# Scalsol/mega.pytorch

Hardware: AMD Instinct MI355X
Metric: frames/sec MEGA R-101 inference, 1000x600 VID clip (higher is better)
Workload: dtype bf16

## Files before the change

mega/pytorch_amd/csrc/bneck64.hip:

```cpp
#include <cstdlib>

#include "common.h"

namespace {

constexpr int BK_TY = 8, BK_TX = 16;
constexpr int BK_PY = BK_TY + 2, BK_PX = BK_TX + 2;
constexpr int BK_NP = BK_PY * BK_PX;
constexpr int BK_M1 = 192;
constexpr int BK_NT = 512;
constexpr int BK_W2ROW = 1168;
constexpr int BK_WROW = 144;
constexpr int BK_SBROW = 528;
constexpr int BK_OFF_W2 = 0;
constexpr int BK_OFF_T1 = 64 * BK_W2ROW;
constexpr int BK_OFF_XB = BK_OFF_T1 + BK_NP * 128;
constexpr int BK_OFF_W1 = BK_OFF_XB + BK_M1 * 128;
constexpr int BK_XB_BYTES = 256 * BK_WROW;
constexpr int BK_OFF_T2 = BK_OFF_XB + BK_XB_BYTES;
constexpr int BK_LDS = BK_OFF_T2 + 128 * 128;
constexpr int BK_OFF_ST = BK_OFF_T1;
static_assert(BK_OFF_ST + 128 * BK_SBROW <= BK_LDS, "staging must fit");
static_assert(BK_M1 * 128 + 64 * BK_WROW <= BK_XB_BYTES, "x chunk + w1 chunk must fit the XB region");

struct Bneck64Params {
  const bf16_t* x;
  const bf16_t* w1;
  const bf16_t* w2;
  const bf16_t* w3;
  const float *s1, *b1, *s2, *b2, *s3, *b3;
  bf16_t* out;
  int N, H, W, tiles_y, tiles_x, ntiles;
};

template <typename HT>
__device__ __forceinline__ f32x16_t bk_mma(f32x16_t acc, const uint4& a, const uint4& b) {
  return Half16<HT>::mfma32(__builtin_bit_cast(u32x4_t, a), __builtin_bit_cast(u32x4_t, b), acc);
}

template <typename HT>
__device__ __forceinline__ unsigned bk_relu_pack(float a, float b) {
  const s16x2_t z = {0, 0};
  return __builtin_bit_cast(unsigned, __builtin_elementwise_max(__builtin_bit_cast(s16x2_t, Half16<HT>::pack2(a, b)), z));
}
template <typename HT>
__device__ __forceinline__ bf16_t bk_relu1(float a) {
  const bf16_t h = Half16<HT>::cvt(a);
  return (short)h < 0 ? (bf16_t)0 : h;
}

template <typename HT>
__global__ __launch_bounds__(BK_NT, 2) void bneck64_kernel(Bneck64Params p) {
  extern __shared__ __attribute__((aligned(16))) unsigned char smem[];
  unsigned char* const w2l = smem + BK_OFF_W2;
  unsigned char* const t1l = smem + BK_OFF_T1;
  unsigned char* const xbl = smem + BK_OFF_XB;
  unsigned char* const w1l = smem + BK_OFF_W1;
  unsigned char* const t2l = smem + BK_OFF_T2;
  unsigned char* const sbl = smem + BK_OFF_ST;
  const int tid = threadIdx.x, lane = tid & 63, wave = tid >> 6;
  const int l31 = lane & 31, h = lane >> 5;

  {
    const uint4* wg = reinterpret_cast<const uint4*>(p.w2);
    for (int e = tid; e < 64 * 72; e += BK_NT) {
      const int n = e / 72, c = e - n * 72;
      *reinterpret_cast<uint4*>(w2l + n * BK_W2ROW + c * 16) = wg[e];
    }
  }

  const unsigned xbytes = (unsigned)((size_t)p.N * p.H * p.W * 512);
  const __amdgpu_buffer_rsrc_t rs_x = __builtin_amdgcn_make_buffer_rsrc(const_cast<bf16_t*>(p.x), 0, (int)xbytes, 0x00020000);
  const __amdgpu_buffer_rsrc_t rs_o = __builtin_amdgcn_make_buffer_rsrc(p.out, 0, (int)xbytes, 0x00020000);
  constexpr unsigned OOB = 0x80000000u;

  auto tile_origin = [&](int t, int& n, int& y0, int& x0) {
    const int per_img = p.tiles_y * p.tiles_x;
    n = t / per_img;
    const int r = t - n * per_img;
    const int ty = r / p.tiles_x;
    y0 = ty * BK_TY;
    x0 = (r - ty * p.tiles_x) * BK_TX;
  };

  u32x4_t px[12], pw1[4];
  auto prefetch = [&](int t) {
    int n, y0, x0;
    const bool live = t < p.ntiles;
    tile_origin(live ? t : 0, n, y0, x0);
    unsigned off[3];
#pragma unroll
    for (int i = 0; i < 3; ++i) {
      const int v = tid + BK_NT * i;
      const int row = v >> 3, j = v & 7;
      const int py = row / BK_PX, pxx = row - py * BK_PX;
      const int yy = y0 - 1 + py, xx = x0 - 1 + pxx;
      const bool ok = live && row < BK_NP && (unsigned)yy < (unsigned)p.H && (unsigned)xx < (unsigned)p.W;
      off[i] = ok ? (unsigned)(((n * p.H + yy) * p.W + xx) * 512 + j * 16) : OOB;
    }
#pragma unroll
    for (int kc = 0; kc < 4; ++kc) {
#pragma unroll
      for (int i = 0; i < 3; ++i) {
        px[3 * kc + i] = __builtin_amdgcn_raw_buffer_load_b128(rs_x, off[i], kc * 128, 0);
      }
      pw1[kc] = *reinterpret_cast<const u32x4_t*>(p.w1 + (tid >> 3) * 256 + kc * 64 + (tid & 7) * 8);
    }
  };

  const int r1 = 32 * wave + l31;
  const unsigned a1_base = (unsigned)(r1 * 128), a1_sw = (unsigned)((r1 >> 1) & 7);
  const unsigned b1_base = (unsigned)(l31 * BK_WROW + h * 16);
  const int mb2 = wave >> 1, nb2 = wave & 1;
  const int ay = 2 * mb2 + (l31 >> 4), ax = l31 & 15;
  const unsigned a2_base = (unsigned)((ay * BK_PX + ax) * 128);
  const int b2_off = (32 * nb2 + l31) * BK_W2ROW + h * 16;
  const unsigned a3_base = (unsigned)(l31 * 128), a3_sw = (unsigned)((l31 >> 1) & 7);
  const unsigned b3_base = (unsigned)((32 * wave + l31) * BK_WROW + h * 16);
  const float s1a = p.s1[l31], s1b = p.s1[32 + l31], b1a = p.b1[l31], b1b = p.b1[32 + l31];
  const float s2v = p.s2[32 * nb2 + l31], b2v = p.b2[32 * nb2 + l31];
  const float s3v = p.s3[32 * wave + l31], b3v = p.b3[32 * wave + l31];

  int t = blockIdx.x;
  prefetch(t);
  __syncthreads();
  for (; t < p.ntiles; t += gridDim.x) {
    int n, y0, x0;
    tile_origin(t, n, y0, x0);
    f32x16_t c1a, c1b;
#pragma unroll
    for (int r = 0; r < 16; ++r) { c1a[r] = 0.f; c1b[r] = 0.f; }
#pragma unroll
    for (int kc = 0; kc < 4; ++kc) {
#pragma unroll
      for (int i = 0; i < 3; ++i) {
        const int v = tid + BK_NT * i;
        const int row = v >> 3, j = v & 7;
        *reinterpret_cast<u32x4_t*>(xbl + row * 128 + ((j ^ ((row >> 1) & 7)) * 16)) = px[3 * kc + i];
      }
      *reinterpret_cast<u32x4_t*>(w1l + (tid >> 3) * BK_WROW + (tid & 7) * 16) = pw1[kc];
      __syncthreads();
      if (wave < 6) {
#pragma unroll
        for (int ks = 0; ks < 4; ++ks) {
          const uint4 a = *reinterpret_cast<const uint4*>(xbl + a1_base + (((unsigned)(2 * ks + h) ^ a1_sw) << 4));
          const uint4 b0 = *reinterpret_cast<const uint4*>(w1l + b1_base + ks * 32);
          const uint4 b1 = *reinterpret_cast<const uint4*>(w1l + 32 * BK_WROW + b1_base + ks * 32);
          c1a = bk_mma<HT>(c1a, a, b0);
          c1b = bk_mma<HT>(c1b, a, b1);
        }
      }
      __syncthreads();
    }
    u32x4_t pw3[4];
#pragma unroll
    for (int i = 0; i < 4; ++i) pw3[i] = reinterpret_cast<const u32x4_t*>(p.w3)[tid + BK_NT * i];
    int ho = h, lo = l31;
    asm volatile("" : "+v"(ho), "+v"(lo));
    if (wave < 6) {
#pragma unroll
      for (int r = 0; r < 16; ++r) {
        const int R = 32 * wave + (r & 3) + 8 * (r >> 2) + 4 * ho;
        if (R < BK_NP) {
          const int py = R / BK_PX, pxx = R - py * BK_PX;
          const int yy = y0 - 1 + py, xx = x0 - 1 + pxx;
          const bool in = (unsigned)yy < (unsigned)p.H && (unsigned)xx < (unsigned)p.W;
          const bf16_t ra = bk_relu1<HT>(c1a[r] * s1a + b1a), rb = bk_relu1<HT>(c1b[r] * s1b + b1b);
          const bf16_t va = in ? ra : (bf16_t)0;
          const bf16_t vb = in ? rb : (bf16_t)0;
          unsigned char* base = t1l + R * 128;
          const int sw = (pxx >> 1) & 7;
          *reinterpret_cast<bf16_t*>(base + (((lo >> 3) ^ sw) * 16) + (lo & 7) * 2) = va;
          *reinterpret_cast<bf16_t*>(base + ((((32 + lo) >> 3) ^ sw) * 16) + (lo & 7) * 2) = vb;
        }
      }
    }
#pragma unroll
    for (int i = 0; i < 4; ++i) {
      const int v = tid + BK_NT * i;
      *reinterpret_cast<u32x4_t*>(xbl + (v >> 3) * BK_WROW + (v & 7) * 16) = pw3[i];
    }
    prefetch(t + gridDim.x);
    __syncthreads();
    f32x16_t c2;
#pragma unroll
    for (int r = 0; r < 16; ++r) c2[r] = 0.f;
#pragma unroll
    for (int kh = 0; kh < 3; ++kh)
#pragma unroll
      for (int kw = 0; kw < 3; ++kw)
#pragma unroll
        for (int ks = 0; ks < 4; ++ks) {
          const unsigned sw2 = (unsigned)(((ax + kw) >> 1) & 7);
          const uint4 a = *reinterpret_cast<const uint4*>(t1l + a2_base + (kh * BK_PX + kw) * 128 +
                                                          (((unsigned)(2 * ks + h) ^ sw2) << 4));
          const uint4 b = *reinterpret_cast<const uint4*>(w2l + b2_off + (kh * 3 + kw) * 128 + ks * 32);
          c2 = bk_mma<HT>(c2, a, b);
        }
    {
      const int c = 32 * nb2 + lo;
#pragma unroll
      for (int r = 0; r < 16; ++r) {
        const int P = 32 * mb2 + (r & 3) + 8 * (r >> 2) + 4 * ho;
        *reinterpret_cast<bf16_t*>(t2l + P * 128 + (((c >> 3) ^ ((P >> 1) & 7)) * 16) + (c & 7) * 2) = bk_relu1<HT>(c2[r] * s2v + b2v);
      }
    }
    __syncthreads();
    unsigned pk[4][8];
    {
      uint4 bf[4];
#pragma unroll
      for (int ks = 0; ks < 4; ++ks) bf[ks] = *reinterpret_cast<const uint4*>(xbl + b3_base + ks * 32);
      const int c3ch = 32 * wave + lo;
      const unsigned res_base = (unsigned)(((n * p.H + y0) * p.W + x0 + 4 * ho) * 512 + c3ch * 2);
#pragma unroll
      for (int mb = 0; mb < 4; ++mb) {
        __builtin_amdgcn_sched_barrier(0);
        float rs[16];
#pragma unroll
        for (int r = 0; r < 16; ++r) {
          const int yy = y0 + 2 * mb + (r >> 3), xx = x0 + (r & 3) + 8 * ((r >> 2) & 1) + 4 * ho;
          const unsigned o = (yy < p.H && xx < p.W) ? res_base : OOB;
          const unsigned short q = __builtin_amdgcn_raw_buffer_load_b16(
              rs_x, o, ((2 * mb + (r >> 3)) * p.W + (r & 3) + 8 * ((r >> 2) & 1)) * 512, 0);
          rs[r] = Half16<HT>::one(q);
        }
        f32x16_t c3;
#pragma unroll
        for (int r = 0; r < 16; ++r) c3[r] = 0.f;
#pragma unroll
        for (int ks = 0; ks < 4; ++ks) {
          const uint4 a = *reinterpret_cast<const uint4*>(t2l + mb * 4096 + a3_base + (((unsigned)(2 * ks + h) ^ a3_sw) << 4));
          c3 = bk_mma<HT>(c3, a, bf[ks]);
        }
#pragma unroll
        for (int q = 0; q < 8; ++q) {
          float v0 = c3[2 * q] * s3v + b3v, v1 = c3[2 * q + 1] * s3v + b3v;
          v0 += rs[2 * q];
          v1 += rs[2 * q + 1];
          pk[mb][q] = bk_relu_pack<HT>(v0, v1);
        }
      }
    }
    __syncthreads();
    {
      const int c3ch = 32 * wave + lo;
#pragma unroll
      for (int mb = 0; mb < 4; ++mb)
#pragma unroll
        for (int r = 0; r < 16; ++r) {
          const int P = 32 * mb + (r & 3) + 8 * (r >> 2) + 4 * ho;
          const unsigned v = pk[mb][r >> 1];
          *reinterpret_cast<bf16_t*>(sbl + P * BK_SBROW + c3ch * 2) = (bf16_t)((r & 1) ? (v >> 16) : (v & 0xffffu));
        }
    }
    __syncthreads();
#pragma unroll
    for (int i = 0; i < 8; ++i) {
      const int id = tid + BK_NT * i;
      const int P = id >> 5, cv = id & 31;
      const int yy = y0 + (P >> 4), xx = x0 + (P & 15);
      const uint4 v = *reinterpret_cast<const uint4*>(sbl + P * BK_SBROW + cv * 16);
      const u32x4_t q = {v.x, v.y, v.z, v.w};
      const unsigned o = (yy < p.H && xx < p.W) ? (unsigned)(((n * p.H + yy) * p.W + xx) * 512 + cv * 16) : OOB;
      __builtin_amdgcn_raw_buffer_store_b128(q, rs_o, o, 0, 0);
    }
    __syncthreads();
  }
}

constexpr int BD_OFF_W2 = 0;
constexpr int BD_OFF_T1 = 64 * BK_W2ROW;
constexpr int BD_OFF_XP = BD_OFF_T1 + BK_NP * 128;
constexpr int BD_OFF_WR = BD_OFF_XP + BK_M1 * 128;
constexpr int BD_LDS = BD_OFF_WR + 256 * BK_WROW;
static_assert(BD_OFF_T1 + 128 * BK_SBROW <= BD_LDS, "output staging must fit over t1 / x patch / weight region");

struct Bneck64DsParams {
  const bf16_t* x;
  const bf16_t* w1;
  const bf16_t* w2;
  const bf16_t* w3;
  const bf16_t* wd;
  const float *s1, *b1, *s2, *b2, *s3, *b3, *sd, *bd;
  bf16_t* out;
  int N, H, W, tiles_y, tiles_x, ntiles;
};

template <typename HT>
__global__ __launch_bounds__(BK_NT, 2) void bneck64_ds_kernel(Bneck64DsParams p) {
  extern __shared__ __attribute__((aligned(16))) unsigned char smem[];
  unsigned char* const w2l = smem + BD_OFF_W2;
  unsigned char* const t1l = smem + BD_OFF_T1;
  unsigned char* const t2l = smem + BD_OFF_T1;
  unsigned char* const xpl = smem + BD_OFF_XP;
  unsigned char* const wrl = smem + BD_OFF_WR;
  unsigned char* const sbl = smem + BD_OFF_T1;
  const int tid = threadIdx.x, lane = tid & 63, wave = tid >> 6;
  const int l31 = lane & 31, h = lane >> 5;
  {
    const uint4* wg = reinterpret_cast<const uint4*>(p.w2);
    for (int e = tid; e < 64 * 72; e += BK_NT) {
      const int n = e / 72, c = e - n * 72;
      *reinterpret_cast<uint4*>(w2l + n * BK_W2ROW + c * 16) = wg[e];
    }
  }
  const unsigned xbytes = (unsigned)((size_t)p.N * p.H * p.W * 128), obytes = (unsigned)((size_t)p.N * p.H * p.W * 512);
  const __amdgpu_buffer_rsrc_t rs_x = __builtin_amdgcn_make_buffer_rsrc(const_cast<bf16_t*>(p.x), 0, (int)xbytes, 0x00020000);
  const __amdgpu_buffer_rsrc_t rs_o = __builtin_amdgcn_make_buffer_rsrc(p.out, 0, (int)obytes, 0x00020000);
  constexpr unsigned OOB = 0x80000000u;
  auto tile_origin = [&](int t, int& n, int& y0, int& x0) {
    const int per_img = p.tiles_y * p.tiles_x;
    n = t / per_img;
    const int r = t - n * per_img;
    const int ty = r / p.tiles_x;
    y0 = ty * BK_TY;
    x0 = (r - ty * p.tiles_x) * BK_TX;
  };
  u32x4_t px[3];
  auto prefetch = [&](int t) {
    int n, y0, x0;
    const bool live = t < p.ntiles;
    tile_origin(live ? t : 0, n, y0, x0);
#pragma unroll
    for (int i = 0; i < 3; ++i) {
      const int v = tid + BK_NT * i;
      const int row = v >> 3, j = v & 7;
      const int py = row / BK_PX, pxx = row - py * BK_PX;
      const int yy = y0 - 1 + py, xx = x0 - 1 + pxx;
      const bool ok = live && row < BK_NP && (unsigned)yy < (unsigned)p.H && (unsigned)xx < (unsigned)p.W;
      px[i] = __builtin_amdgcn_raw_buffer_load_b128(rs_x, ok ? (unsigned)(((n * p.H + yy) * p.W + xx) * 128 + j * 16) : OOB, 0, 0);
    }
  };
  const int r1 = 32 * wave + l31;
  const unsigned a1_base = (unsigned)(r1 * 128), a1_sw = (unsigned)((r1 >> 1) & 7);
  const unsigned bw_base = (unsigned)(l31 * BK_WROW + h * 16);
  const int mb2 = wave >> 1, nb2 = wave & 1;
  const int ay = 2 * mb2 + (l31 >> 4), ax = l31 & 15;
  const unsigned a2_base = (unsigned)((ay * BK_PX + ax) * 128);
  const int b2_off = (32 * nb2 + l31) * BK_W2ROW + h * 16;
  const unsigned a3_base = (unsigned)(l31 * 128), a3_sw = (unsigned)((l31 >> 1) & 7);
  const float s1a = p.s1[l31], s1b = p.s1[32 + l31], b1a = p.b1[l31], b1b = p.b1[32 + l31];
  const float s2v = p.s2[32 * nb2 + l31], b2v = p.b2[32 * nb2 + l31];
  const float s3v = p.s3[32 * wave + l31], b3v = p.b3[32 * wave + l31];
  const float sdv = p.sd[32 * wave + l31], bdv = p.bd[32 * wave + l31];

  int t = blockIdx.x;
  prefetch(t);
  __syncthreads();
  for (; t < p.ntiles; t += gridDim.x) {
    int n, y0, x0;
    tile_origin(t, n, y0, x0);
    int ho = h, lo = l31;
    asm volatile("" : "+v"(ho), "+v"(lo));
#pragma unroll
    for (int i = 0; i < 3; ++i) {
      const int v = tid + BK_NT * i;
      const int row = v >> 3, j = v & 7;
      *reinterpret_cast<u32x4_t*>(xpl + row * 128 + ((j ^ ((row >> 1) & 7)) * 16)) = px[i];
    }
    *reinterpret_cast<u32x4_t*>(wrl + (tid >> 3) * BK_WROW + (tid & 7) * 16) =
        *reinterpret_cast<const u32x4_t*>(p.w1 + (tid >> 3) * 64 + (tid & 7) * 8);
    u32x4_t pwd[4];
#pragma unroll
    for (int i = 0; i < 4; ++i) pwd[i] = reinterpret_cast<const u32x4_t*>(p.wd)[tid + BK_NT * i];
    __syncthreads();
    f32x16_t c1a, c1b;
#pragma unroll
    for (int r = 0; r < 16; ++r) { c1a[r] = 0.f; c1b[r] = 0.f; }
    if (wave < 6) {
#pragma unroll
      for (int ks = 0; ks < 4; ++ks) {
        const uint4 a = *reinterpret_cast<const uint4*>(xpl + a1_base + (((unsigned)(2 * ks + h) ^ a1_sw) << 4));
        const uint4 b0 = *reinterpret_cast<const uint4*>(wrl + bw_base + ks * 32);
        const uint4 b1 = *reinterpret_cast<const uint4*>(wrl + 32 * BK_WROW + bw_base + ks * 32);
        c1a = bk_mma<HT>(c1a, a, b0);
        c1b = bk_mma<HT>(c1b, a, b1);
      }
#pragma unroll
      for (int r = 0; r < 16; ++r) {
        const int R = 32 * wave + (r & 3) + 8 * (r >> 2) + 4 * ho;
        if (R < BK_NP) {
          const int py = R / BK_PX, pxx = R - py * BK_PX;
          const int yy = y0 - 1 + py, xx = x0 - 1 + pxx;
          const bool in = (unsigned)yy < (unsigned)p.H && (unsigned)xx < (unsigned)p.W;
          const bf16_t ra = bk_relu1<HT>(c1a[r] * s1a + b1a), rb = bk_relu1<HT>(c1b[r] * s1b + b1b);
          const bf16_t va = in ? ra : (bf16_t)0;
          const bf16_t vb = in ? rb : (bf16_t)0;
          unsigned char* base = t1l + R * 128;
          const int sw = (pxx >> 1) & 7;
          *reinterpret_cast<bf16_t*>(base + (((lo >> 3) ^ sw) * 16) + (lo & 7) * 2) = va;
          *reinterpret_cast<bf16_t*>(base + ((((32 + lo) >> 3) ^ sw) * 16) + (lo & 7) * 2) = vb;
        }
      }
    }
    __syncthreads();
#pragma unroll
    for (int i = 0; i < 4; ++i) {
      const int v = tid + BK_NT * i;
      *reinterpret_cast<u32x4_t*>(wrl + (v >> 3) * BK_WROW + (v & 7) * 16) = pwd[i];
    }
    u32x4_t pw3[4];
#pragma unroll
    for (int i = 0; i < 4; ++i) pw3[i] = reinterpret_cast<const u32x4_t*>(p.w3)[tid + BK_NT * i];
    prefetch(t + gridDim.x);
    f32x16_t c2;
#pragma unroll
    for (int r = 0; r < 16; ++r) c2[r] = 0.f;
#pragma unroll
    for (int kh = 0; kh < 3; ++kh)
#pragma unroll
      for (int kw = 0; kw < 3; ++kw)
#pragma unroll
        for (int ks = 0; ks < 4; ++ks) {
          const unsigned sw2 = (unsigned)(((ax + kw) >> 1) & 7);
          const uint4 a = *reinterpret_cast<const uint4*>(t1l + a2_base + (kh * BK_PX + kw) * 128 +
                                                          (((unsigned)(2 * ks + h) ^ sw2) << 4));
          const uint4 b = *reinterpret_cast<const uint4*>(w2l + b2_off + (kh * 3 + kw) * 128 + ks * 32);
          c2 = bk_mma<HT>(c2, a, b);
        }
    __syncthreads();
    {
      const int c = 32 * nb2 + lo;
#pragma unroll
      for (int r = 0; r < 16; ++r) {
        const int P = 32 * mb2 + (r & 3) + 8 * (r >> 2) + 4 * ho;
        *reinterpret_cast<bf16_t*>(t2l + P * 128 + (((c >> 3) ^ ((P >> 1) & 7)) * 16) + (c & 7) * 2) = bk_relu1<HT>(c2[r] * s2v + b2v);
      }
    }
    unsigned pk[4][8];
    {
      uint4 bf[4];
#pragma unroll
      for (int ks = 0; ks < 4; ++ks) bf[ks] = *reinterpret_cast<const uint4*>(wrl + 32 * wave * BK_WROW + bw_base + ks * 32);
#pragma unroll
      for (int mb = 0; mb < 4; ++mb) {
        const int R = (2 * mb + (l31 >> 4) + 1) * BK_PX + (l31 & 15) + 1;
        const unsigned xa = (unsigned)(R * 128), xs = (unsigned)((R >> 1) & 7);
        f32x16_t cd;
#pragma unroll
        for (int r = 0; r < 16; ++r) cd[r] = 0.f;
#pragma unroll
        for (int ks = 0; ks < 4; ++ks) {
          const uint4 a = *reinterpret_cast<const uint4*>(xpl + xa + (((unsigned)(2 * ks + h) ^ xs) << 4));
          cd = bk_mma<HT>(cd, a, bf[ks]);
        }
#pragma unroll
        for (int q = 0; q < 8; ++q) pk[mb][q] = Half16<HT>::pack2(cd[2 * q] * sdv + bdv, cd[2 * q + 1] * sdv + bdv);
      }
    }
    __syncthreads();
#pragma unroll
    for (int i = 0; i < 4; ++i) {
      const int v = tid + BK_NT * i;
      *reinterpret_cast<u32x4_t*>(wrl + (v >> 3) * BK_WROW + (v & 7) * 16) = pw3[i];
    }
    __syncthreads();
    {
      uint4 bf[4];
#pragma unroll
      for (int ks = 0; ks < 4; ++ks) bf[ks] = *reinterpret_cast<const uint4*>(wrl + 32 * wave * BK_WROW + bw_base + ks * 32);
#pragma unroll
      for (int mb = 0; mb < 4; ++mb) {
        f32x16_t c3;
#pragma unroll
        for (int r = 0; r < 16; ++r) c3[r] = 0.f;
#pragma unroll
        for (int ks = 0; ks < 4; ++ks) {
          const uint4 a = *reinterpret_cast<const uint4*>(t2l + mb * 4096 + a3_base + (((unsigned)(2 * ks + h) ^ a3_sw) << 4));
          c3 = bk_mma<HT>(c3, a, bf[ks]);
        }
#pragma unroll
        for (int q = 0; q < 8; ++q) {
          float v0 = c3[2 * q] * s3v + b3v, v1 = c3[2 * q + 1] * s3v + b3v;
          v0 += Half16<HT>::lo(pk[mb][q]);
          v1 += Half16<HT>::hi(pk[mb][q]);
          pk[mb][q] = bk_relu_pack<HT>(v0, v1);
        }
      }
    }
    __syncthreads();
    {
      const int c3ch = 32 * wave + lo;
#pragma unroll
      for (int mb = 0; mb < 4; ++mb)
#pragma unroll
        for (int r = 0; r < 16; ++r) {
          const int P = 32 * mb + (r & 3) + 8 * (r >> 2) + 4 * ho;
          const unsigned v = pk[mb][r >> 1];
          *reinterpret_cast<bf16_t*>(sbl + P * BK_SBROW + c3ch * 2) = (bf16_t)((r & 1) ? (v >> 16) : (v & 0xffffu));
        }
    }
    __syncthreads();
#pragma unroll
    for (int i = 0; i < 8; ++i) {
      const int id = tid + BK_NT * i;
      const int P = id >> 5, cv = id & 31;
      const int yy = y0 + (P >> 4), xx = x0 + (P & 15);
      const uint4 v = *reinterpret_cast<const uint4*>(sbl + P * BK_SBROW + cv * 16);
      const u32x4_t q = {v.x, v.y, v.z, v.w};
      const unsigned o = (yy < p.H && xx < p.W) ? (unsigned)(((n * p.H + yy) * p.W + xx) * 512 + cv * 16) : OOB;
      __builtin_amdgcn_raw_buffer_store_b128(q, rs_o, o, 0, 0);
    }
    __syncthreads();
  }
}

}

extern "C" int mega_bottleneck64_fwd_dt(const void* x, const void* w1, const float* s1, const float* b1, const void* w2,
                                        const float* s2, const float* b2, const void* w3, const float* s3, const float* b3,
                                        void* out, int N, int H, int W, int dtype, void* stream) {
  mega_clear_error();
  if (dtype != MEGA_BF16 && dtype != MEGA_F16) return MEGA_ERR_ARG;
  if (!x || !w1 || !s1 || !b1 || !w2 || !s2 || !b2 || !w3 || !s3 || !b3 || !out || N <= 0 || H <= 0 || W <= 0) return MEGA_ERR_ARG;
  if ((size_t)N * H * W * 256 * 2 >= 0x7FF00000ull) return MEGA_ERR_ARG;
  Bneck64Params p;
  p.x = (const bf16_t*)x; p.w1 = (const bf16_t*)w1; p.w2 = (const bf16_t*)w2; p.w3 = (const bf16_t*)w3;
  p.s1 = s1; p.b1 = b1; p.s2 = s2; p.b2 = b2; p.s3 = s3; p.b3 = b3;
  p.out = (bf16_t*)out;
  p.N = N; p.H = H; p.W = W;
  p.tiles_y = cdiv(H, BK_TY);
  p.tiles_x = cdiv(W, BK_TX);
  const long tiles = (long)N * p.tiles_y * p.tiles_x;
  if (tiles > 0x7FFFFFFF) return MEGA_ERR_ARG;
  p.ntiles = (int)tiles;
  int cus = 256;
  {
    static int cached[64] = {0};
    int dev = 0, n = 0;
    if (hipGetDevice(&dev) != hipSuccess || dev < 0 || dev >= 64) dev = 0;
    if (!cached[dev]) {
      if (hipDeviceGetAttribute(&n, hipDeviceAttributeMultiprocessorCount, dev) == hipSuccess && n > 0) cached[dev] = n;
      else cached[dev] = 256;
    }
    cus = cached[dev];
  }
  const int grid = (int)(tiles < cus ? tiles : cus);
  if (dtype == MEGA_F16) {
    (void)hipFuncSetAttribute((const void*)bneck64_kernel<f16_t>, hipFuncAttributeMaxDynamicSharedMemorySize, BK_LDS);
    hipLaunchKernelGGL(bneck64_kernel<f16_t>, dim3(grid), dim3(BK_NT), BK_LDS, (hipStream_t)stream, p);
  } else {
    (void)hipFuncSetAttribute((const void*)bneck64_kernel<bf16_t>, hipFuncAttributeMaxDynamicSharedMemorySize, BK_LDS);
    hipLaunchKernelGGL(bneck64_kernel<bf16_t>, dim3(grid), dim3(BK_NT), BK_LDS, (hipStream_t)stream, p);
  }
  return mega_check_launch();
}

extern "C" int mega_bottleneck64_ds_fwd_dt(const void* x, const void* w1, const float* s1, const float* b1, const void* w2,
                                           const float* s2, const float* b2, const void* w3, const float* s3, const float* b3,
                                           const void* wd, const float* sd, const float* bd, void* out, int N, int H, int W,
                                           int dtype, void* stream) {
  mega_clear_error();
  if (dtype != MEGA_BF16 && dtype != MEGA_F16) return MEGA_ERR_ARG;
  if (!x || !w1 || !s1 || !b1 || !w2 || !s2 || !b2 || !w3 || !s3 || !b3 || !wd || !sd || !bd || !out || N <= 0 || H <= 0 || W <= 0)
    return MEGA_ERR_ARG;
  if ((size_t)N * H * W * 256 * 2 >= 0x7FF00000ull) return MEGA_ERR_ARG;
  Bneck64DsParams p;
  p.x = (const bf16_t*)x; p.w1 = (const bf16_t*)w1; p.w2 = (const bf16_t*)w2; p.w3 = (const bf16_t*)w3; p.wd = (const bf16_t*)wd;
  p.s1 = s1; p.b1 = b1; p.s2 = s2; p.b2 = b2; p.s3 = s3; p.b3 = b3; p.sd = sd; p.bd = bd;
  p.out = (bf16_t*)out;
  p.N = N; p.H = H; p.W = W;
  p.tiles_y = cdiv(H, BK_TY);
  p.tiles_x = cdiv(W, BK_TX);
  const long tiles = (long)N * p.tiles_y * p.tiles_x;
  if (tiles > 0x7FFFFFFF) return MEGA_ERR_ARG;
  p.ntiles = (int)tiles;
  int cus = 256;
  {
    static int cached[64] = {0};
    int dev = 0, n = 0;
    if (hipGetDevice(&dev) != hipSuccess || dev < 0 || dev >= 64) dev = 0;
    if (!cached[dev]) {
      if (hipDeviceGetAttribute(&n, hipDeviceAttributeMultiprocessorCount, dev) == hipSuccess && n > 0) cached[dev] = n;
      else cached[dev] = 256;
    }
    cus = cached[dev];
  }
  const int grid = (int)(tiles < cus ? tiles : cus);
  if (dtype == MEGA_F16) {
    (void)hipFuncSetAttribute((const void*)bneck64_ds_kernel<f16_t>, hipFuncAttributeMaxDynamicSharedMemorySize, BD_LDS);
    hipLaunchKernelGGL(bneck64_ds_kernel<f16_t>, dim3(grid), dim3(BK_NT), BD_LDS, (hipStream_t)stream, p);
  } else {
    (void)hipFuncSetAttribute((const void*)bneck64_ds_kernel<bf16_t>, hipFuncAttributeMaxDynamicSharedMemorySize, BD_LDS);
    hipLaunchKernelGGL(bneck64_ds_kernel<bf16_t>, dim3(grid), dim3(BK_NT), BD_LDS, (hipStream_t)stream, p);
  }
  return mega_check_launch();
}
```

Baseline: 902.8.

## Swap MFMA operand order and vectorise epilogues with LDS scale/bias and slab output

Swaps the A/B operands of every MFMA so accumulators come out channel-contiguous per lane. The bf16 epilogues for t1, t2 and the downsample path can then write packed 8-byte words instead of scalar 2-byte stores. Per-channel scale/bias vectors move into LDS, either as padding in the w2 rows or in dedicated regions, and are read as float4. w3 and wd fragments now load straight from global memory into registers instead of being staged through LDS. In the main kernel, the residual is read with 16-byte buffer loads instead of 2-byte ones, and the output goes through two fp32 LDS slabs with lighter barriers before 128-bit stores. The intent is fewer LDS and global transactions and fewer barriers, in exchange for more LDS space and more register pressure from the extra accumulators and prefetched residuals.

Result: faster. 921.2 (median of 4 runs) (+2.0%).

```diff
diff --git a/mega/pytorch_amd/csrc/bneck64.hip b/mega/pytorch_amd/csrc/bneck64.hip
--- a/mega/pytorch_amd/csrc/bneck64.hip
+++ b/mega/pytorch_amd/csrc/bneck64.hip
@@ -3,6 +3,8 @@
 #include "common.h"
 
 namespace {
+
+typedef unsigned int u32x2_t __attribute__((ext_vector_type(2)));
 
 constexpr int BK_TY = 8, BK_TX = 16;
 constexpr int BK_PY = BK_TY + 2, BK_PX = BK_TX + 2;
@@ -18,9 +20,12 @@
 constexpr int BK_OFF_W1 = BK_OFF_XB + BK_M1 * 128;
 constexpr int BK_XB_BYTES = 256 * BK_WROW;
 constexpr int BK_OFF_T2 = BK_OFF_XB + BK_XB_BYTES;
-constexpr int BK_LDS = BK_OFF_T2 + 128 * 128;
+constexpr int BK_OFF_SB3 = BK_OFF_T2 + 128 * 128;
+constexpr int BK_LDS = BK_OFF_SB3 + 2 * 256 * 4;
 constexpr int BK_OFF_ST = BK_OFF_T1;
-static_assert(BK_OFF_ST + 128 * BK_SBROW <= BK_LDS, "staging must fit");
+constexpr int BK_SLROW = (256 + 4) * 4;
+constexpr int BK_SLAB = 32 * BK_SLROW;
+static_assert(BK_OFF_ST + 2 * BK_SLAB <= BK_LDS, "the two slabs must fit");
 static_assert(BK_M1 * 128 + 64 * BK_WROW <= BK_XB_BYTES, "x chunk + w1 chunk must fit the XB region");
 
 struct Bneck64Params {
@@ -43,10 +48,58 @@
   const s16x2_t z = {0, 0};
   return __builtin_bit_cast(unsigned, __builtin_elementwise_max(__builtin_bit_cast(s16x2_t, Half16<HT>::pack2(a, b)), z));
 }
+
+constexpr int BK_W2PAD = 576 * 2;
+__device__ __forceinline__ f32x4_t bk_sb12(const unsigned char* w2l, int q) {
+  return *reinterpret_cast<const f32x4_t*>(w2l + q * BK_W2ROW + BK_W2PAD);
+}
+__device__ __forceinline__ void bk_sb12_fill(unsigned char* w2l, int tid, const float* s1, const float* b1, const float* s2, const float* b2) {
+  if (tid < 256) {
+    const float* const src = tid < 64 ? s1 : (tid < 128 ? b1 : (tid < 192 ? s2 : b2));
+    *reinterpret_cast<float*>(w2l + (tid >> 2) * BK_W2ROW + BK_W2PAD + (tid & 3) * 4) = src[tid & 63];
+  }
+}
+
 template <typename HT>
-__device__ __forceinline__ bf16_t bk_relu1(float a) {
-  const bf16_t h = Half16<HT>::cvt(a);
-  return (short)h < 0 ? (bf16_t)0 : h;
+__device__ __forceinline__ void bk_store_t1(unsigned char* t1l, const unsigned char* w2l, const f32x16_t& ca, const f32x16_t& cb,
+                                            int R, int hh, int y0, int x0, int H, int W) {
+  if (R >= BK_NP) return;
+  const int py = R / BK_PX, pxx = R - py * BK_PX;
+  const int yy = y0 - 1 + py, xx = x0 - 1 + pxx;
+  const bool in = (unsigned)yy < (unsigned)H && (unsigned)xx < (unsigned)W;
+  const int sw = (pxx >> 1) & 7;
+  unsigned char* const base = t1l + R * 128 + hh * 8;
+#pragma unroll
+  for (int half = 0; half < 2; ++half)
+#pragma unroll
+    for (int g = 0; g < 4; ++g) {
+      const f32x16_t& c = half ? cb : ca;
+      const f32x4_t sc = bk_sb12(w2l, 8 * half + 2 * g + hh), bi = bk_sb12(w2l, 16 + 8 * half + 2 * g + hh);
+      const unsigned q0 = bk_relu_pack<HT>(fmaf(c[4 * g], sc[0], bi[0]), fmaf(c[4 * g + 1], sc[1], bi[1]));
+      const unsigned q1 = bk_relu_pack<HT>(fmaf(c[4 * g + 2], sc[2], bi[2]), fmaf(c[4 * g + 3], sc[3], bi[3]));
+      const u32x2_t q = {in ? q0 : 0u, in ? q1 : 0u};
+      *reinterpret_cast<u32x2_t*>(base + (((4 * half + g) ^ sw) * 16)) = q;
+    }
+}
+
+template <typename HT>
+__device__ __forceinline__ void bk_store_t2(unsigned char* t2l, const unsigned char* w2l, const f32x16_t& c, int P, int nb, int hh) {
+  unsigned char* const base = t2l + P * 128 + hh * 8;
+  const int sw = (P >> 1) & 7;
+#pragma unroll
+  for (int g = 0; g < 4; ++g) {
+    const f32x4_t sc = bk_sb12(w2l, 32 + 8 * nb + 2 * g + hh), bi = bk_sb12(w2l, 48 + 8 * nb + 2 * g + hh);
+    const u32x2_t q = {bk_relu_pack<HT>(fmaf(c[4 * g], sc[0], bi[0]), fmaf(c[4 * g + 1], sc[1], bi[1])),
+                       bk_relu_pack<HT>(fmaf(c[4 * g + 2], sc[2], bi[2]), fmaf(c[4 * g + 3], sc[3], bi[3]))};
+    *reinterpret_cast<u32x2_t*>(base + (((4 * nb + g) ^ sw) * 16)) = q;
+  }
+}
+
+__device__ __forceinline__ void bk_lds_barrier() {
+  asm volatile("s_waitcnt lgkmcnt(0)" ::: "memory");
+  __builtin_amdgcn_sched_barrier(0);
+  __builtin_amdgcn_s_barrier();
+  asm volatile("" ::: "memory");
 }
 
 template <typename HT>
@@ -67,6 +120,7 @@
       const int n = e / 72, c = e - n * 72;
       *reinterpret_cast<uint4*>(w2l + n * BK_W2ROW + c * 16) = wg[e];
     }
+    bk_sb12_fill(w2l, tid, p.s1, p.b1, p.s2, p.b2);
   }
 
   const unsigned xbytes = (unsigned)((size_t)p.N * p.H * p.W * 512);
@@ -116,10 +170,11 @@
   const unsigned a2_base = (unsigned)((ay * BK_PX + ax) * 128);
   const int b2_off = (32 * nb2 + l31) * BK_W2ROW + h * 16;
   const unsigned a3_base = (unsigned)(l31 * 128), a3_sw = (unsigned)((l31 >> 1) & 7);
-  const unsigned b3_base = (unsigned)((32 * wave + l31) * BK_WROW + h * 16);
-  const float s1a = p.s1[l31], s1b = p.s1[32 + l31], b1a = p.b1[l31], b1b = p.b1[32 + l31];
-  const float s2v = p.s2[32 * nb2 + l31], b2v = p.b2[32 * nb2 + l31];
-  const float s3v = p.s3[32 * wave + l31], b3v = p.b3[32 * wave + l31];
+  const int cv3 = tid & 31, col3 = tid >> 5;
+  if (tid < 256) {
+    reinterpret_cast<float*>(smem + BK_OFF_SB3)[tid] = p.s3[tid];
+    reinterpret_cast<float*>(smem + BK_OFF_SB3)[256 + tid] = p.b3[tid];
+  }
 
   int t = blockIdx.x;
   prefetch(t);
@@ -127,6 +182,8 @@
   for (; t < p.ntiles; t += gridDim.x) {
     int n, y0, x0;
     tile_origin(t, n, y0, x0);
+    const unsigned io_base = (unsigned)(((n * p.H + y0) * p.W + x0 + col3) * 512 + cv3 * 16);
+    const bool io_col = x0 + col3 < p.W;
     f32x16_t c1a, c1b;
 #pragma unroll
     for (int r = 0; r < 16; ++r) { c1a[r] = 0.f; c1b[r] = 0.f; }
@@ -146,40 +203,22 @@
           const uint4 a = *reinterpret_cast<const uint4*>(xbl + a1_base + (((unsigned)(2 * ks + h) ^ a1_sw) << 4));
           const uint4 b0 = *reinterpret_cast<const uint4*>(w1l + b1_base + ks * 32);
           const uint4 b1 = *reinterpret_cast<const uint4*>(w1l + 32 * BK_WROW + b1_base + ks * 32);
-          c1a = bk_mma<HT>(c1a, a, b0);
-          c1b = bk_mma<HT>(c1b, a, b1);
+          c1a = bk_mma<HT>(c1a, b0, a);
+          c1b = bk_mma<HT>(c1b, b1, a);
         }
       }
       __syncthreads();
     }
-    u32x4_t pw3[4];
-#pragma unroll
-    for (int i = 0; i < 4; ++i) pw3[i] = reinterpret_cast<const u32x4_t*>(p.w3)[tid + BK_NT * i];
+    u32x4_t rres[8];
+#pragma unroll
+    for (int i = 0; i < 8; ++i)
+      rres[i] = __builtin_amdgcn_raw_buffer_load_b128(rs_x, (io_col && y0 + i < p.H) ? io_base : OOB, i * p.W * 512, 0);
+    u32x4_t bf3[4];
+#pragma unroll
+    for (int ks = 0; ks < 4; ++ks) bf3[ks] = *reinterpret_cast<const u32x4_t*>(p.w3 + (32 * wave + l31) * 64 + h * 8 + ks * 16);
     int ho = h, lo = l31;
     asm volatile("" : "+v"(ho), "+v"(lo));
-    if (wave < 6) {
-#pragma unroll
-      for (int r = 0; r < 16; ++r) {
-        const int R = 32 * wave + (r & 3) + 8 * (r >> 2) + 4 * ho;
-        if (R < BK_NP) {
-          const int py = R / BK_PX, pxx = R - py * BK_PX;
-          const int yy = y0 - 1 + py, xx = x0 - 1 + pxx;
-          const bool in = (unsigned)yy < (unsigned)p.H && (unsigned)xx < (unsigned)p.W;
-          const bf16_t ra = bk_relu1<HT>(c1a[r] * s1a + b1a), rb = bk_relu1<HT>(c1b[r] * s1b + b1b);
-          const bf16_t va = in ? ra : (bf16_t)0;
-          const bf16_t vb = in ? rb : (bf16_t)0;
-          unsigned char* base = t1l + R * 128;
-          const int sw = (pxx >> 1) & 7;
-          *reinterpret_cast<bf16_t*>(base + (((lo >> 3) ^ sw) * 16) + (lo & 7) * 2) = va;
-          *reinterpret_cast<bf16_t*>(base + ((((32 + lo) >> 3) ^ sw) * 16) + (lo & 7) * 2) = vb;
-        }
-      }
-    }
-#pragma unroll
-    for (int i = 0; i < 4; ++i) {
-      const int v = tid + BK_NT * i;
-      *reinterpret_cast<u32x4_t*>(xbl + (v >> 3) * BK_WROW + (v & 7) * 16) = pw3[i];
-    }
+    if (wave < 6) bk_store_t1<HT>(t1l, w2l, c1a, c1b, 32 * wave + lo, ho, y0, x0, p.H, p.W);
     prefetch(t + gridDim.x);
     __syncthreads();
     f32x16_t c2;
@@ -195,77 +234,71 @@
           const uint4 a = *reinterpret_cast<const uint4*>(t1l + a2_base + (kh * BK_PX + kw) * 128 +
                                                           (((unsigned)(2 * ks + h) ^ sw2) << 4));
           const uint4 b = *reinterpret_cast<const uint4*>(w2l + b2_off + (kh * 3 + kw) * 128 + ks * 32);
-          c2 = bk_mma<HT>(c2, a, b);
-        }
-    {
-      const int c = 32 * nb2 + lo;
-#pragma unroll
-      for (int r = 0; r < 16; ++r) {
-        const int P = 32 * mb2 + (r & 3) + 8 * (r >> 2) + 4 * ho;
-        *reinterpret_cast<bf16_t*>(t2l + P * 128 + (((c >> 3) ^ ((P >> 1) & 7)) * 16) + (c & 7) * 2) = bk_relu1<HT>(c2[r] * s2v + b2v);
-      }
-    }
-    __syncthreads();
-    unsigned pk[4][8];
+          c2 = bk_mma<HT>(c2, b, a);
+        }
+    bk_store_t2<HT>(t2l, w2l, c2, 32 * mb2 + lo, nb2, ho);
+    __syncthreads();
+    f32x16_t c3[4];
     {
       uint4 bf[4];
 #pragma unroll
-      for (int ks = 0; ks < 4; ++ks) bf[ks] = *reinterpret_cast<const uint4*>(xbl + b3_base + ks * 32);
-      const int c3ch = 32 * wave + lo;
-      const unsigned res_base = (unsigned)(((n * p.H + y0) * p.W + x0 + 4 * ho) * 512 + c3ch * 2);
+      for (int ks = 0; ks < 4; ++ks) bf[ks] = __builtin_bit_cast(uint4, bf3[ks]);
 #pragma unroll
       for (int mb = 0; mb < 4; ++mb) {
-        __builtin_amdgcn_sched_barrier(0);
-        float rs[16];
-#pragma unroll
-        for (int r = 0; r < 16; ++r) {
-          const int yy = y0 + 2 * mb + (r >> 3), xx = x0 + (r & 3) + 8 * ((r >> 2) & 1) + 4 * ho;
-          const unsigned o = (yy < p.H && xx < p.W) ? res_base : OOB;
-          const unsigned short q = __builtin_amdgcn_raw_buffer_load_b16(
-              rs_x, o, ((2 * mb + (r >> 3)) * p.W + (r & 3) + 8 * ((r >> 2) & 1)) * 512, 0);
-          rs[r] = Half16<HT>::one(q);
-        }
-        f32x16_t c3;
-#pragma unroll
-        for (int r = 0; r < 16; ++r) c3[r] = 0.f;
+#pragma unroll
+        for (int r = 0; r < 16; ++r) c3[mb][r] = 0.f;
 #pragma unroll
         for (int ks = 0; ks < 4; ++ks) {
           const uint4 a = *reinterpret_cast<const uint4*>(t2l + mb * 4096 + a3_base + (((unsigned)(2 * ks + h) ^ a3_sw) << 4));
-          c3 = bk_mma<HT>(c3, a, bf[ks]);
-        }
-#pragma unroll
-        for (int q = 0; q < 8; ++q) {
-          float v0 = c3[2 * q] * s3v + b3v, v1 = c3[2 * q + 1] * s3v + b3v;
-          v0 += rs[2 * q];
-          v1 += rs[2 * q + 1];
-          pk[mb][q] = bk_relu_pack<HT>(v0, v1);
+          c3[mb] = bk_mma<HT>(c3[mb], bf[ks], a);
         }
       }
     }
     __syncthreads();
     {
-      const int c3ch = 32 * wave + lo;
-#pragma unroll
-      for (int mb = 0; mb < 4; ++mb)
-#pragma unroll
-        for (int r = 0; r < 16; ++r) {
-          const int P = 32 * mb + (r & 3) + 8 * (r >> 2) + 4 * ho;
-          const unsigned v = pk[mb][r >> 1];
-          *reinterpret_cast<bf16_t*>(sbl + P * BK_SBROW + c3ch * 2) = (bf16_t)((r & 1) ? (v >> 16) : (v & 0xffffu));
-        }
-    }
-    __syncthreads();
-#pragma unroll
-    for (int i = 0; i < 8; ++i) {
-      const int id = tid + BK_NT * i;
-      const int P = id >> 5, cv = id & 31;
-      const int yy = y0 + (P >> 4), xx = x0 + (P & 15);
-      const uint4 v = *reinterpret_cast<const uint4*>(sbl + P * BK_SBROW + cv * 16);
-      const u32x4_t q = {v.x, v.y, v.z, v.w};
-      const unsigned o = (yy < p.H && xx < p.W) ? (unsigned)(((n * p.H + yy) * p.W + xx) * 512 + cv * 16) : OOB;
-      __builtin_amdgcn_raw_buffer_store_b128(q, rs_o, o, 0, 0);
-    }
-    __syncthreads();
+      int slab1 = BK_SLAB;
+      asm volatile("" : "+v"(slab1));
+      float s3r[8], b3r[8];
+      {
+        const f32x4_t* const sb = reinterpret_cast<const f32x4_t*>(smem + BK_OFF_SB3) + 2 * cv3;
+        const f32x4_t sa = sb[0], sc = sb[1], ba = sb[64], bc = sb[65];
+#pragma unroll
+        for (int u = 0; u < 4; ++u) { s3r[u] = sa[u]; s3r[4 + u] = sc[u]; b3r[u] = ba[u]; b3r[4 + u] = bc[u]; }
+      }
+#pragma unroll
+      for (int mb = 0; mb < 4; ++mb) {
+        unsigned char* const sl = (mb & 1) ? sbl + slab1 : sbl;
+        {
+          unsigned char* const dst = sl + l31 * BK_SLROW + (32 * wave + 4 * h) * 4;
+#pragma unroll
+          for (int g = 0; g < 4; ++g) {
+            const f32x4_t q = {c3[mb][4 * g], c3[mb][4 * g + 1], c3[mb][4 * g + 2], c3[mb][4 * g + 3]};
+            *reinterpret_cast<f32x4_t*>(dst + g * 32) = q;
+          }
+        }
+        bk_lds_barrier();
+#pragma unroll
+        for (int it = 0; it < 2; ++it) {
+          const int i = 2 * mb + it;
+          const unsigned char* const src = sl + (16 * it + col3) * BK_SLROW + cv3 * 32;
+          const f32x4_t q0 = *reinterpret_cast<const f32x4_t*>(src), q1 = *reinterpret_cast<const f32x4_t*>(src + 16);
+          float v[8];
+#pragma unroll
+          for (int u = 0; u < 4; ++u) { v[u] = fmaf(q0[u], s3r[u], b3r[u]); v[4 + u] = fmaf(q1[u], s3r[4 + u], b3r[4 + u]); }
+          u32x4_t r4 = rres[i];
+          asm volatile("" : "+v"(r4));
+          u32x4_t o;
+#pragma unroll
+          for (int d = 0; d < 4; ++d) {
+            v[2 * d] += Half16<HT>::lo(r4[d]);
+            v[2 * d + 1] += Half16<HT>::hi(r4[d]);
+            o[d] = bk_relu_pack<HT>(v[2 * d], v[2 * d + 1]);
+          }
+          __builtin_amdgcn_raw_buffer_store_b128(o, rs_o, (io_col && y0 + i < p.H) ? io_base : OOB, i * p.W * 512, 0);
+        }
+      }
+    }
+    bk_lds_barrier();
   }
 }
 
@@ -273,8 +306,9 @@
 constexpr int BD_OFF_T1 = 64 * BK_W2ROW;
 constexpr int BD_OFF_XP = BD_OFF_T1 + BK_NP * 128;
 constexpr int BD_OFF_WR = BD_OFF_XP + BK_M1 * 128;
-constexpr int BD_LDS = BD_OFF_WR + 256 * BK_WROW;
-static_assert(BD_OFF_T1 + 128 * BK_SBROW <= BD_LDS, "output staging must fit over t1 / x patch / weight region");
+constexpr int BD_OFF_SB = BD_OFF_T1 + 128 * BK_SBROW;
+constexpr int BD_LDS = BD_OFF_SB + 4 * 256 * 4;
+static_assert(BD_OFF_WR + 64 * BK_WROW <= BD_OFF_SB, "w1 must end before the scale / bias vectors");
 
 struct Bneck64DsParams {
   const bf16_t* x;
@@ -304,6 +338,7 @@
       const int n = e / 72, c = e - n * 72;
       *reinterpret_cast<uint4*>(w2l + n * BK_W2ROW + c * 16) = wg[e];
     }
+    bk_sb12_fill(w2l, tid, p.s1, p.b1, p.s2, p.b2);
   }
   const unsigned xbytes = (unsigned)((size_t)p.N * p.H * p.W * 128), obytes = (unsigned)((size_t)p.N * p.H * p.W * 512);
   const __amdgpu_buffer_rsrc_t rs_x = __builtin_amdgcn_make_buffer_rsrc(const_cast<bf16_t*>(p.x), 0, (int)xbytes, 0x00020000);
@@ -339,11 +374,11 @@
   const int ay = 2 * mb2 + (l31 >> 4), ax = l31 & 15;
   const unsigned a2_base = (unsigned)((ay * BK_PX + ax) * 128);
   const int b2_off = (32 * nb2 + l31) * BK_W2ROW + h * 16;
-  const unsigned a3_base = (unsigned)(l31 * 128), a3_sw = (unsigned)((l31 >> 1) & 7);
-  const float s1a = p.s1[l31], s1b = p.s1[32 + l31], b1a = p.b1[l31], b1b = p.b1[32 + l31];
-  const float s2v = p.s2[32 * nb2 + l31], b2v = p.b2[32 * nb2 + l31];
-  const float s3v = p.s3[32 * wave + l31], b3v = p.b3[32 * wave + l31];
-  const float sdv = p.sd[32 * wave + l31], bdv = p.bd[32 * wave + l31];
+  if (tid < 256) {
+    float* const sb = reinterpret_cast<float*>(smem + BD_OFF_SB);
+    sb[tid] = p.sd[tid]; sb[256 + tid] = p.bd[tid]; sb[512 + tid] = p.s3[tid]; sb[768 + tid] = p.b3[tid];
+  }
+  const f32x4_t* const sbv = reinterpret_cast<const f32x4_t*>(smem + BD_OFF_SB) + 8 * wave + h;
 
   int t = blockIdx.x;
   prefetch(t);
@@ -361,9 +396,9 @@
     }
     *reinterpret_cast<u32x4_t*>(wrl + (tid >> 3) * BK_WROW + (tid & 7) * 16) =
         *reinterpret_cast<const u32x4_t*>(p.w1 + (tid >> 3) * 64 + (tid & 7) * 8);
-    u32x4_t pwd[4];
-#pragma unroll
-    for (int i = 0; i < 4; ++i) pwd[i] = reinterpret_cast<const u32x4_t*>(p.wd)[tid + BK_NT * i];
+    u32x4_t bfd[4];
+#pragma unroll
+    for (int ks = 0; ks < 4; ++ks) bfd[ks] = *reinterpret_cast<const u32x4_t*>(p.wd + (32 * wave + l31) * 64 + h * 8 + ks * 16);
     __syncthreads();
     f32x16_t c1a, c1b;
 #pragma unroll
@@ -374,35 +409,15 @@
         const uint4 a = *reinterpret_cast<const uint4*>(xpl + a1_base + (((unsigned)(2 * ks + h) ^ a1_sw) << 4));
         const uint4 b0 = *reinterpret_cast<const uint4*>(wrl + bw_base + ks * 32);
         const uint4 b1 = *reinterpret_cast<const uint4*>(wrl + 32 * BK_WROW + bw_base + ks * 32);
-        c1a = bk_mma<HT>(c1a, a, b0);
-        c1b = bk_mma<HT>(c1b, a, b1);
-      }
-#pragma unroll
-      for (int r = 0; r < 16; ++r) {
-        const int R = 32 * wave + (r & 3) + 8 * (r >> 2) + 4 * ho;
-        if (R < BK_NP) {
-          const int py = R / BK_PX, pxx = R - py * BK_PX;
-          const int yy = y0 - 1 + py, xx = x0 - 1 + pxx;
-          const bool in = (unsigned)yy < (unsigned)p.H && (unsigned)xx < (unsigned)p.W;
-          const bf16_t ra = bk_relu1<HT>(c1a[r] * s1a + b1a), rb = bk_relu1<HT>(c1b[r] * s1b + b1b);
-          const bf16_t va = in ? ra : (bf16_t)0;
-          const bf16_t vb = in ? rb : (bf16_t)0;
-          unsigned char* base = t1l + R * 128;
-          const int sw = (pxx >> 1) & 7;
-          *reinterpret_cast<bf16_t*>(base + (((lo >> 3) ^ sw) * 16) + (lo & 7) * 2) = va;
-          *reinterpret_cast<bf16_t*>(base + ((((32 + lo) >> 3) ^ sw) * 16) + (lo & 7) * 2) = vb;
-        }
-      }
-    }
-    __syncthreads();
-#pragma unroll
-    for (int i = 0; i < 4; ++i) {
-      const int v = tid + BK_NT * i;
-      *reinterpret_cast<u32x4_t*>(wrl + (v >> 3) * BK_WROW + (v & 7) * 16) = pwd[i];
-    }
-    u32x4_t pw3[4];
-#pragma unroll
-    for (int i = 0; i < 4; ++i) pw3[i] = reinterpret_cast<const u32x4_t*>(p.w3)[tid + BK_NT * i];
+        c1a = bk_mma<HT>(c1a, b0, a);
+        c1b = bk_mma<HT>(c1b, b1, a);
+      }
+      bk_store_t1<HT>(t1l, w2l, c1a, c1b, 32 * wave + lo, ho, y0, x0, p.H, p.W);
+    }
+    __syncthreads();
+    u32x4_t bf3[4];
+#pragma unroll
+    for (int ks = 0; ks < 4; ++ks) bf3[ks] = *reinterpret_cast<const u32x4_t*>(p.w3 + (32 * wave + l31) * 64 + h * 8 + ks * 16);
     prefetch(t + gridDim.x);
     f32x16_t c2;
 #pragma unroll
@@ -417,49 +432,40 @@
           const uint4 a = *reinterpret_cast<const uint4*>(t1l + a2_base + (kh * BK_PX + kw) * 128 +
                                                           (((unsigned)(2 * ks + h) ^ sw2) << 4));
           const uint4 b = *reinterpret_cast<const uint4*>(w2l + b2_off + (kh * 3 + kw) * 128 + ks * 32);
-          c2 = bk_mma<HT>(c2, a, b);
-        }
-    __syncthreads();
-    {
-      const int c = 32 * nb2 + lo;
-#pragma unroll
-      for (int r = 0; r < 16; ++r) {
-        const int P = 32 * mb2 + (r & 3) + 8 * (r >> 2) + 4 * ho;
-        *reinterpret_cast<bf16_t*>(t2l + P * 128 + (((c >> 3) ^ ((P >> 1) & 7)) * 16) + (c & 7) * 2) = bk_relu1<HT>(c2[r] * s2v + b2v);
-      }
-    }
+          c2 = bk_mma<HT>(c2, b, a);
+        }
+    __syncthreads();
+    bk_store_t2<HT>(t2l, w2l, c2, 32 * mb2 + lo, nb2, ho);
     unsigned pk[4][8];
     {
       uint4 bf[4];
 #pragma unroll
-      for (int ks = 0; ks < 4; ++ks) bf[ks] = *reinterpret_cast<const uint4*>(wrl + 32 * wave * BK_WROW + bw_base + ks * 32);
+      for (int ks = 0; ks < 4; ++ks) bf[ks] = __builtin_bit_cast(uint4, bfd[ks]);
 #pragma unroll
       for (int mb = 0; mb < 4; ++mb) {
-        const int R = (2 * mb + (l31 >> 4) + 1) * BK_PX + (l31 & 15) + 1;
+        const int R = (2 * mb + (lo >> 4) + 1) * BK_PX + (lo & 15) + 1;
         const unsigned xa = (unsigned)(R * 128), xs = (unsigned)((R >> 1) & 7);
         f32x16_t cd;
 #pragma unroll
         for (int r = 0; r < 16; ++r) cd[r] = 0.f;
 #pragma unroll
         for (int ks = 0; ks < 4; ++ks) {
-          const uint4 a = *reinterpret_cast<const uint4*>(xpl + xa + (((unsigned)(2 * ks + h) ^ xs) << 4));
-          cd = bk_mma<HT>(cd, a, bf[ks]);
-        }
-#pragma unroll
-        for (int q = 0; q < 8; ++q) pk[mb][q] = Half16<HT>::pack2(cd[2 * q] * sdv + bdv, cd[2 * q + 1] * sdv + bdv);
-      }
-    }
-    __syncthreads();
-#pragma unroll
-    for (int i = 0; i < 4; ++i) {
-      const int v = tid + BK_NT * i;
-      *reinterpret_cast<u32x4_t*>(wrl + (v >> 3) * BK_WROW + (v & 7) * 16) = pw3[i];
+          const uint4 a = *reinterpret_cast<const uint4*>(xpl + xa + (((unsigned)(2 * ks + ho) ^ xs) << 4));
+          cd = bk_mma<HT>(cd, bf[ks], a);
+        }
+#pragma unroll
+        for (int g = 0; g < 4; ++g) {
+          const f32x4_t sc = sbv[2 * g], bi = sbv[64 + 2 * g];
+          pk[mb][2 * g] = Half16<HT>::pack2(fmaf(cd[4 * g], sc[0], bi[0]), fmaf(cd[4 * g + 1], sc[1], bi[1]));
+          pk[mb][2 * g + 1] = Half16<HT>::pack2(fmaf(cd[4 * g + 2], sc[2], bi[2]), fmaf(cd[4 * g + 3], sc[3], bi[3]));
+        }
+      }
     }
     __syncthreads();
     {
       uint4 bf[4];
 #pragma unroll
-      for (int ks = 0; ks < 4; ++ks) bf[ks] = *reinterpret_cast<const uint4*>(wrl + 32 * wave * BK_WROW + bw_base + ks * 32);
+      for (int ks = 0; ks < 4; ++ks) bf[ks] = __builtin_bit_cast(uint4, bf3[ks]);
 #pragma unroll
       for (int mb = 0; mb < 4; ++mb) {
         f32x16_t c3;
@@ -467,28 +473,31 @@
         for (int r = 0; r < 16; ++r) c3[r] = 0.f;
 #pragma unroll
         for (int ks = 0; ks < 4; ++ks) {
-          const uint4 a = *reinterpret_cast<const uint4*>(t2l + mb * 4096 + a3_base + (((unsigned)(2 * ks + h) ^ a3_sw) << 4));
-          c3 = bk_mma<HT>(c3, a, bf[ks]);
-        }
-#pragma unroll
-        for (int q = 0; q < 8; ++q) {
-          float v0 = c3[2 * q] * s3v + b3v, v1 = c3[2 * q + 1] * s3v + b3v;
-          v0 += Half16<HT>::lo(pk[mb][q]);
-          v1 += Half16<HT>::hi(pk[mb][q]);
-          pk[mb][q] = bk_relu_pack<HT>(v0, v1);
+          const uint4 a = *reinterpret_cast<const uint4*>(t2l + mb * 4096 + lo * 128 + (((unsigned)(2 * ks + ho) ^ (unsigned)((lo >> 1) & 7)) << 4));
+          c3 = bk_mma<HT>(c3, bf[ks], a);
+        }
+#pragma unroll
+        for (int g = 0; g < 4; ++g) {
+          const f32x4_t sc = sbv[128 + 2 * g], bi = sbv[192 + 2 * g];
+#pragma unroll
+          for (int d = 0; d < 2; ++d) {
+            float v0 = fmaf(c3[4 * g + 2 * d], sc[2 * d], bi[2 * d]), v1 = fmaf(c3[4 * g + 2 * d + 1], sc[2 * d + 1], bi[2 * d + 1]);
+            v0 += Half16<HT>::lo(pk[mb][2 * g + d]);
+            v1 += Half16<HT>::hi(pk[mb][2 * g + d]);
+            pk[mb][2 * g + d] = bk_relu_pack<HT>(v0, v1);
+          }
         }
       }
     }
     __syncthreads();
     {
-      const int c3ch = 32 * wave + lo;
+      unsigned char* const dst = sbl + lo * BK_SBROW + (32 * wave + 4 * ho) * 2;
 #pragma unroll
       for (int mb = 0; mb < 4; ++mb)
 #pragma unroll
-        for (int r = 0; r < 16; ++r) {
-          const int P = 32 * mb + (r & 3) + 8 * (r >> 2) + 4 * ho;
-          const unsigned v = pk[mb][r >> 1];
-          *reinterpret_cast<bf16_t*>(sbl + P * BK_SBROW + c3ch * 2) = (bf16_t)((r & 1) ? (v >> 16) : (v & 0xffffu));
+        for (int g = 0; g < 4; ++g) {
+          const u32x2_t q = {pk[mb][2 * g], pk[mb][2 * g + 1]};
+          *reinterpret_cast<u32x2_t*>(dst + mb * 32 * BK_SBROW + g * 16) = q;
         }
     }
     __syncthreads();
```
